# TheCacophonyProject/audio-analysis

Hardware: AMD Instinct MI355X
Metric: audio-seconds classified/sec/GPU on 60 s mono; max|delta logit| vs CPU ref (higher is better)
Workload: dtype bf16x3; 1 GPU; config2: 64 windows/step (39 of clip A + 25 of clip B, 60 s 48 kHz mono), htk log-mel n_fft 4096 hop 640 160 mel + model1 CNN; model=model1, global_batch=64, seq_len=144000, parallelism=dp1, pipeline=2 batches in flight on 2 streams, clip_pairs=4 resident clip pairs in rotation, one per step

## Files before the change

audio-analysis_amd/csrc/aa_cnn.hip:

```cpp
#include "aa_common.h"

#include <cmath>
#include <cstdlib>
#include <cstring>
#include <string>
#include <type_traits>
#include <vector>

namespace aa {

typedef __attribute__((ext_vector_type(8))) __bf16 bf16x8;
typedef __attribute__((ext_vector_type(4))) float f32x4;
typedef __attribute__((ext_vector_type(2))) float f32x2;
typedef __attribute__((ext_vector_type(16))) float f32x16;
typedef __bf16 bf16;
struct fp8 {
    uint8_t v;
};
struct bf16x3 {};

template <typename T>
struct Prec {
    using L = T;
    using G = T;
// ... 801 lines not shown
        for (int dx = 0; dx < pw; ++dx) {
            const int h = oh * ph + dy, x = ow * pw + dx;
            float acc[8];
#pragma unroll
            for (int o = 0; o < 8; ++o) acc[o] = 0.f;
            for (int i = 0; i < kh; ++i)
                for (int j = 0; j < kw; ++j) {
                    const TI* src = img + ((size_t)(h + i) * Win + x + j) * cin;
                    const float* wk = w + (size_t)c0 * K + (i * kw + j) * cin;
                    for (int c = 0; c < cin; ++c) {
                        float v = to_f(src[c]);
                        if (has_mag) v = powf(v, mag_exp);
#pragma unroll
                        for (int o = 0; o < 8; ++o)
                            if (o < nc) acc[o] = fmaf(v, wk[(size_t)o * K + c], acc[o]);
                    }
                }
#pragma unroll
            for (int o = 0; o < 8; ++o)
                if (o < nc) best[o] = fmaxf(best[o], apply_act(acc[o] + bias[c0 + o], act, alpha));
        }
    TO* dst = out + ((size_t)(n * Hout + oh) * Wout + ow) * cout + c0;
    for (int o = 0; o < nc; ++o) dst[o] = to_t<TO>(best[o]);
}

template <typename TI>
__global__ __launch_bounds__(256) void pool_dense(const TI* __restrict__ in, int HW, int C,
                                                  const float* __restrict__ w, const float* __restrict__ b, int U,
                                                  int sigmoid, float* __restrict__ logits, float* __restrict__ probs) {
    extern __shared__ float mx[];
    const int n = blockIdx.x;
    const TI* src = in + (size_t)n * HW * C;
    for (int c = threadIdx.x; c < C; c += blockDim.x) {
        float m = -INFINITY;
        for (int p = 0; p < HW; ++p) m = fmaxf(m, to_f(src[(size_t)p * C + c]));
        mx[c] = m;
    }
    __syncthreads();
    for (int u = threadIdx.x; u < U; u += blockDim.x) {
        float v;
        if (w) {
            v = 0.f;
            for (int c = 0; c < C; ++c) v = fmaf(mx[c], w[(size_t)c * U + u], v);
            v += b[u];
        } else {
            v = mx[u];
        }
        logits[(size_t)n * U + u] = v;
        if (probs) probs[(size_t)n * U + u] = sigmoid ? 1.f / (1.f + expf(-v)) : v;
    }
}

__global__ void track_mean(const float* __restrict__ probs, int n_models, long long model_stride, int L,
                           const int* __restrict__ wb, const int* __restrict__ wc,
                           float* __restrict__ out) {
    const int t = blockIdx.x;
    const int c = threadIdx.x;
    if (c >= L) return;
    constexpr int U = 40;
    float acc = 0.f;
    const int n = wc[t];
    const float* base = probs + (size_t)wb[t] * L + c;
    for (int w0 = 0; w0 < n; w0 += U) {
        float m[U];
#pragma unroll
        for (int u = 0; u < U; ++u) m[u] = 0.f;
        for (int k = 0; k < n_models; ++k) {
            float v[U];
#pragma unroll
            for (int u = 0; u < U; ++u) v[u] = base[k * model_stride + (size_t)min(w0 + u, n - 1) * L];
#pragma unroll
            for (int u = 0; u < U; ++u) m[u] = __fadd_rn(m[u], v[u]);
        }
#pragma unroll
        for (int u = 0; u < U; ++u)
            if (w0 + u < n) acc = __fadd_rn(acc, __fdiv_rn(m[u], (float)n_models));
    }
    out[(size_t)t * L + c] = n > 0 ? __fdiv_rn(acc, (float)n) : NAN;
}

}

#include "aa_conv_x3.h"
#include "aa_conv_wg.h"
#include "aa_gconv.h"
#include "aa_conv_tail.h"

namespace aa {

template <int MODE>
__global__ void stage_decode(const void* __restrict__ src, float* __restrict__ dst, size_t total, int cout) {
    for (size_t i = (size_t)blockIdx.x * blockDim.x + threadIdx.x; i < total; i += (size_t)gridDim.x * blockDim.x) {
        float v;
        if (MODE == 0) {
            v = static_cast<const float*>(src)[i];
        } else if (MODE == 1) {
            v = __uint_as_float((uint32_t) static_cast<const uint16_t*>(src)[i] << 16);
        } else if (MODE == 2) {
            const uint32_t b = static_cast<const uint8_t*>(src)[i];
            const int e = (b >> 3) & 15, m = b & 7;
            const float a = (e == 15 && m == 7) ? __uint_as_float(0x7fc00000u)
                            : e == 0            ? ldexpf((float)m, -9)
                                                : ldexpf((float)(8 + m), e - 10);
            v = (b & 0x80) ? -a : a;
        } else {
            const size_t pix = i / (size_t)cout;
            const int c = (int)(i - pix * (size_t)cout);
            const uint16_t* h = static_cast<const uint16_t*>(src) + pix * (size_t)cout * 2 + (size_t)(c >> 5) * 64 + (c & 31);
            v = __uint_as_float((uint32_t)h[0] << 16) + __uint_as_float((uint32_t)h[32] << 16);
        }
        dst[i] = v;
    }
}

}

#include "aa_cnn_plan.h"

namespace aa {

template <typename Launch>
static int launch_tuned(const Stage& s, const Stage* first, int n, const void* kernel, size_t lds, bool window32,
                        int pool, int th, int tw, int bn, Launch&& launch) {
    if (window32)
        AA_CHECK((double)s.Hin * s.Win * s.cin * 4 < 2147483647.0, AA_ERR_UNSUPPORTED,
                 "conv %s: one window's activations exceed 2 GiB", s.name.c_str());
    FirstConv fc{};
    if (first) {
        const float slope = first->act == ACT_LEAKY ? first->alpha : first->act == ACT_RELU ? 0.f : 1.f;
        fc = FirstConv{(const float*)first->d_w, first->d_b, first->act, slope, first->has_mag,
                       first->mag_exp, first->Hin, first->Win, s.lm_f16};
    }
    AA_CHECK(lds <= 160 * 1024, AA_ERR_UNSUPPORTED, "conv %s: %zu B LDS", s.name.c_str(), lds);
    AA_DYN_LDS(kernel, lds);
    const int tiles_h = (s.Hout * pool + th - 1) / th;
    const int tiles_w = (s.Wout * pool + tw - 1) / tw;
    launch(dim3(tiles_h * tiles_w, s.cout_pad / bn, n), tiles_w, fc);
    AA_LAUNCH_CHECK();
    return AA_OK;
}

template <typename T, int KH, int KW, int CIN, int WM, int WN, int MF, int NF, int POOL, int TH, int TW,
          bool FUSED = false, bool EBF16 = false, int OCC = 0>
static int launch_mfma(const Stage& s, const void* in, void* out, int n, hipStream_t st,
                       const Stage* first = nullptr) {
    auto k = conv_mfma<T, KH, KW, CIN, WM, WN, MF, NF, POOL, TH, TW, FUSED, 0, EBF16, OCC>;
    constexpr int BN = WN * NF * 16;
    const size_t lds = conv_lds_bytes<T, KH, KW, CIN, BN, TH, TW, FUSED, EBF16>();
    using GT = typename Prec<T>::G;
    using LT = typename Prec<T>::L;
    return launch_tuned(s, FUSED ? first : nullptr, n, (const void*)k, lds, false, POOL, TH, TW, BN,
                        [&](dim3 grid, int tiles_w, const FirstConv& fc) {
        hipLaunchKernelGGL(k, grid, dim3(WM * WN * 64), lds, st, (const GT*)in, s.Hin, s.Win, (const LT*)s.d_w, s.d_b,
                           (GT*)out, s.Hout, s.Wout, s.cout, tiles_w, s.act, s.alpha, fc);
    });
}

template <int KH, int KW, int CIN, int WM, int WN, int MF, int NF, int POOL, int TH, int TW, bool RING, bool AJIT,
          int OCC, bool FUSED, bool IN_SPLIT, bool OUT_SPLIT>
static int launch_x3(const Stage& s, const void* in, void* out, int n, hipStream_t st, const Stage* first) {
    auto k = conv_x3<KH, KW, CIN, WM, WN, MF, NF, POOL, TH, TW, FUSED, 0, RING, AJIT, OCC, IN_SPLIT, OUT_SPLIT>;
    constexpr int BN = WN * NF * 16;
    const size_t lds = x3_lds_bytes<KH, KW, CIN, BN, TH, TW, FUSED, RING>();
    return launch_tuned(s, FUSED ? first : nullptr, n, (const void*)k, lds, true, POOL, TH, TW, BN,
                        [&](dim3 grid, int tiles_w, const FirstConv& fc) {
        hipLaunchKernelGGL(k, grid, dim3(WM * WN * 64), lds, st, (const float*)in, s.Hin, s.Win, (const bf16*)s.d_w,
                           s.d_b, (float*)out, s.Hout, s.Wout, s.cout, tiles_w, s.act, s.alpha, fc);
    });
}

template <int KH, int CIN, int WM, int WN, int MF, int NF, int POOL, int TH, int TW, int OCC, int WO, int NPASS,
          int BD, int SLIDE, bool IN_SPLIT, bool OUT_SPLIT>
static int launch_wg(const Stage& s, const void* in, void* out, int n, hipStream_t st) {
    auto k = conv_wg<KH, CIN, WM, WN, MF, NF, POOL, TH, TW, OCC, IN_SPLIT, OUT_SPLIT, 0, WO, NPASS, BD, SLIDE>;
    constexpr int BN = WN * NF * 16;
    const size_t lds = wg_lds_bytes<KH, BN, TH, TW, WO, NPASS, WN>();
    return launch_tuned(s, nullptr, n, (const void*)k, lds, true, POOL, TH, TW, BN,
                        [&](dim3 grid, int tiles_w, const FirstConv&) {
        hipLaunchKernelGGL(k, grid, dim3(WM * WN * 64), lds, st, (const float*)in, s.Hin, s.Win, (const bf16*)s.d_w,
                           s.d_b, (float*)out, s.Hout, s.Wout, s.cout, tiles_w, s.act, s.alpha);
    });
}

template <bool CAN_FUSE, typename F>
static int dispatch_split(const Stage& s, F&& f) {
    using Y = std::true_type;
    using N = std::false_type;
    if constexpr (CAN_FUSE) {
        if (s.fused_first) return s.out_split ? f(Y{}, N{}, Y{}) : f(Y{}, N{}, N{});
    }
    if (s.in_split) return s.out_split ? f(N{}, Y{}, Y{}) : f(N{}, Y{}, N{});
    return s.out_split ? f(N{}, N{}, Y{}) : f(N{}, N{}, N{});
}

template <typename T>
static int launch_stage(const Model& m, const Stage& s, const void* in, void* out, float* logits,
                        float* probs, int n, hipStream_t st, const Stage* first, float* tmp) {
    using GT = typename Prec<T>::G;
    if (s.kind == ST_SMALL) {
        dim3 grid((s.Hc * s.Wc + 255) / 256, n);
        hipLaunchKernelGGL((conv_small<GT, 3, 3, 32>), grid, dim3(256), 0, st, (const float*)in, s.Hin,
                           s.Win, (const float*)s.d_w, s.d_b, s.has_mag, s.mag_exp, (GT*)out, s.Hc, s.Wc,
                           s.act, s.alpha);
        AA_LAUNCH_CHECK();
        return AA_OK;
    }
    if (s.kind == ST_GCONV) {
        if constexpr (!is_split<T>()) {
            set_error("%s: the runtime-shaped MFMA conv is split-bf16 only", s.name.c_str());
            return AA_ERR_UNSUPPORTED;
        } else {
            const ConvGeom g{s.Hin, s.Win, s.cin, s.Hc, s.Wc, s.cout, s.kh, s.kw, 1, 1, 0, 0, s.cin_pad};
            const bool pooled = s.ph > 1 || s.pw > 1;
            float* conv_out = pooled ? tmp : static_cast<float*>(out);
            const int gact_ = s.act == ACT_LEAKY ? GACT_LEAKY : s.act == ACT_RELU ? GACT_RELU : GACT_NONE;
            hipLaunchKernelGGL((gconv_x3t<2, 2, 2, 2>), dim3((s.Hc * s.Wc + 63) / 64, s.cout_pad / 64, n), dim3(256), 0, st,
                               (const float*)in, (const uint16_t*)s.d_w, s.d_b, conv_out, g, s.cout_pad, gact_,
                               s.alpha, nullptr, nullptr);
            AA_LAUNCH_CHECK();
            if (pooled) {
                const size_t items = (size_t)s.Hout * s.Wout * s.cout;
                hipLaunchKernelGGL(gpool2d, dim3((unsigned)((items + 255) / 256), n), dim3(256), 0, st, tmp,
                                   (float*)out, s.Hc, s.Wc, s.cout, s.Hout, s.Wout, s.ph, s.pw, s.ph, s.pw, 0, 0, 0,
                                   GACT_NONE, 0.f);
                AA_LAUNCH_CHECK();
            }
            return AA_OK;
        }
    }
    if (s.kind == ST_GENERIC) {
        if constexpr (is_fp8<T>()) {
            set_error("%s: no fp8 kernel for this shape", s.name.c_str());
            return AA_ERR_UNSUPPORTED;
        } else {
            dim3 grid((s.Hout * s.Wout + 255) / 256, (s.cout + 7) / 8, n);
            if (s.is_first) {
                hipLaunchKernelGGL((conv_generic<float, GT>), grid, dim3(256), 0, st, (const float*)in, s.Hin,
                                   s.Win, s.cin, (const float*)s.d_w, s.d_b, s.kh, s.kw, s.cout, s.ph, s.pw, s.Hout,
                                   s.Wout, s.act, s.alpha, s.has_mag, s.mag_exp, (GT*)out);
            } else {
                hipLaunchKernelGGL((conv_generic<GT, GT>), grid, dim3(256), 0, st, (const GT*)in, s.Hin, s.Win,
                                   s.cin, (const float*)s.d_w, s.d_b, s.kh, s.kw, s.cout, s.ph, s.pw, s.Hout,
                                   s.Wout, s.act, s.alpha, 0, 1.f, (GT*)out);
            }
            AA_LAUNCH_CHECK();
            return AA_OK;
        }
    }
    if (s.kind == ST_POOLDENSE) {
        hipLaunchKernelGGL((pool_dense<GT>), dim3(n), dim3(256), (size_t)s.cin * sizeof(float), st, (const GT*)in,
                           s.Hin * s.Win, s.cin, (const float*)s.d_w, s.d_b, s.cout, s.sigmoid, logits, probs);
        AA_LAUNCH_CHECK();
        return AA_OK;
    }
    if (s.kind == ST_HEAD && s.tail) {
        if constexpr (is_split<T>()) {
            const Stage& c = *first;
            const int tiles_h = (c.Hc + TAIL_TH - 1) / TAIL_TH, tiles_w = (c.Wc + TAIL_TW - 1) / TAIL_TW;
            auto k = conv_tail_x3<1, 3, 128, AA_TAIL_MF, TAIL_TH, TAIL_TW>;
            constexpr size_t lds = tail_lds_bytes<1, 3, 128, TAIL_TH, TAIL_TW>();
            AA_DYN_LDS(k, lds);
            float* part = static_cast<float*>(out);
            hipLaunchKernelGGL(k, dim3(tiles_h * tiles_w, 1, n), dim3(TAIL_NW * 64), lds, st, (const float*)in, c.Hin,
                               c.Win, (const bf16*)c.d_w, c.d_b, c.Hc, c.Wc, tiles_w, c.act, c.alpha,
                               (const bf16*)s.d_tw, part);
            AA_LAUNCH_CHECK();
            hipLaunchKernelGGL(head_final, dim3(n), dim3(64), 0, st, part, tiles_h * tiles_w, 32, s.d_b, s.cout, s.act,
                               s.alpha, s.sigmoid, logits, probs, (const float*)nullptr);
            AA_LAUNCH_CHECK();
            return AA_OK;
        } else {
            set_error("%s: the fused tail is split-bf16 only", s.name.c_str());
            return AA_ERR_UNSUPPORTED;
        }
    }
    if (s.kind == ST_HEAD) {
        const int HW = s.Hin * s.Win, parts = (HW + 63) / 64;
        float* part = static_cast<float*>(out);
        const float* hsc = is_fp8<T>() ? s.d_b + s.cout_pad : nullptr;
        hipLaunchKernelGGL((conv_head<GT, 1, 2>), dim3(n, parts, s.cout_pad / 32), dim3(256), 0, st, (const GT*)in,
                           HW, s.cin, (const GT*)s.d_w, s.d_b, s.cout, s.act, s.alpha, s.sigmoid, logits, probs, part,
                           hsc);
        AA_LAUNCH_CHECK();
        hipLaunchKernelGGL(head_final, dim3(n), dim3(s.cout <= 64 ? 64 : 256), 0, st, part, parts, s.cout_pad, s.d_b,
                           s.cout, s.act, s.alpha, s.sigmoid, logits, probs, hsc);
        AA_LAUNCH_CHECK();
        return AA_OK;
    }
    if (s.fused_first) {
        AA_CHECK(s.kh == 3 && s.kw == 3 && s.cin == 32 && s.pool == 3, AA_ERR_UNSUPPORTED,
                 "no fused first-layer kernel for %s", s.name.c_str());
    }
    if constexpr (is_split<T>()) {
        if (s.wg) {
#define AA_LAUNCHW(KH, CIN, POOL, WM, WN, MF, NF, TH, TW, OCC, WO, NPASS, BD, SLIDE)                             \
            if (s.kh == KH && s.cin == CIN && s.pool == POOL)                                                    \
                return dispatch_split<false>(s, [&](auto, auto is, auto os) {                                    \
                    return launch_wg<KH, CIN, WM, WN, MF, NF, POOL, TH, TW, OCC, WO, NPASS, BD, SLIDE,           \
                                     decltype(is)::value, decltype(os)::value>(s, in, out, n, st);               \
                });
            AA_WG_CFGS(AA_LAUNCHW)
#undef AA_LAUNCHW
            set_error("conv %dx%d cin %d pool %d: no Winograd kernel instantiation", s.kh, s.kw, s.cin, s.pool);
            return AA_ERR_UNSUPPORTED;
        }
#define AA_LAUNCH3(KH, KW, CIN, POOL, WM, WN, MF, NF, TH, TW, RING, AJIT, OCC)                                   \
        if (s.kh == KH && s.kw == KW && s.cin == CIN && s.pool == POOL)                                          \
            return dispatch_split<CIN == 32 && KH == 3 && KW == 3>(s, [&](auto fu, auto is, auto os) {           \
                return launch_x3<KH, KW, CIN, WM, WN, MF, NF, POOL, TH, TW, RING, AJIT, OCC, decltype(fu)::value, \
                                 decltype(is)::value, decltype(os)::value>(s, in, out, n, st, first);            \
            });
        AA_X3_CFGS(AA_LAUNCH3)
#undef AA_LAUNCH3
        set_error("conv %dx%d cin %d pool %d: no split-bf16 kernel instantiation", s.kh, s.kw, s.cin, s.pool);
        return AA_ERR_UNSUPPORTED;
    }
#define AA_LAUNCH(T_, KH, KW, CIN, POOL, WM, WN, MF, NF, TH, TW, EB, OCC)                                        \
    if constexpr (std::is_same<T, T_>::value) {                                                          \
        if (s.kh == KH && s.kw == KW && s.cin == CIN && s.pool == POOL) {                                \
            if (s.fused_first) {                                                                         \
                if constexpr (CIN == 32 && KH == 3 && KW == 3)                                           \
                    return launch_mfma<T, KH, KW, CIN, WM, WN, MF, NF, POOL, TH, TW, true, EB, OCC>(s, in, out, \
                                                                                              n, st, first); \
            } else {                                                                                     \
                return launch_mfma<T, KH, KW, CIN, WM, WN, MF, NF, POOL, TH, TW, false, EB, OCC>(s, in, out, n, st); \
            }                                                                                            \
        }                                                                                                \
    }
    AA_CONV_CFGS(AA_LAUNCH)
#undef AA_LAUNCH
    set_error("conv %dx%d cin %d pool %d: no kernel instantiation", s.kh, s.kw, s.cin, s.pool);
    return AA_ERR_UNSUPPORTED;
}

static void free_model(Model* m) {
    if (!m) return;
    m->timer.release();
    if (m->uploaded)
        for (auto& s : m->st) {
            (void)hipFree(s.d_w);
            (void)hipFree(s.d_b);
            (void)hipFree(s.d_tw);
        }
    delete m;
}

static int upload_model(Model* m) {
    m->uploaded = true;
    auto put = [](void** d, const void* h, size_t bytes) {
        hipError_t e = hipMalloc(d, bytes ? bytes : 4);
        if (e == hipSuccess && bytes) e = hipMemcpy(*d, h, bytes, hipMemcpyHostToDevice);
        return e;
    };
    for (Stage& s : m->st) {
        hipError_t e = s.h_w.empty() ? hipSuccess : put(&s.d_w, s.h_w.data(), s.h_w.size());
        if (e == hipSuccess) e = put((void**)&s.d_b, s.h_b.data(), sizeof(float) * s.h_b.size());
        AA_CHECK(e == hipSuccess, AA_ERR_HIP, "aa_model_create: layer %d: %s", s.layer_end, hipGetErrorString(e));
        if (!s.h_tw.empty()) e = put(&s.d_tw, s.h_tw.data(), s.h_tw.size());
        AA_CHECK(e == hipSuccess, AA_ERR_HIP, "aa_model_create: %s", hipGetErrorString(e));
        std::vector<uint8_t>().swap(s.h_w);
        std::vector<uint8_t>().swap(s.h_tw);
        std::vector<float>().swap(s.h_b);
    }
    return AA_OK;
}

template <typename T>
static int run_stages_t(Model* m, const void* x, int n, int last_stage, float* logits, float* probs, void* workspace,
                        hipStream_t st, bool timed, const void** last_out) {
    const size_t es = prec_bytes(m->prec);
    char* buf[2] = {static_cast<char*>(workspace),
                    static_cast<char*>(workspace) + align_up(m->act_elems[0] * es * n, 256)};
    float* tmp = reinterpret_cast<float*>(buf[1] + align_up(m->act_elems[1] * es * n, 256));
    const void* in = x;
    for (int k = 0; k <= last_stage; ++k) {
        const Stage& s = m->st[k];
        if (s.skipped) continue;
        void* out = buf[(s.tail ? k - 1 : k) % 2];
        const Stage* first = (s.fused_first || s.tail) ? &m->st[k - 1] : nullptr;
        hipEvent_t e0 = nullptr;
        int rc = timed ? m->timer.begin(k, st, &e0) : AA_OK;
        if (rc != AA_OK) return rc;
        rc = launch_stage<T>(*m, s, in, out, logits, probs, n, st, first, tmp);
        if (rc != AA_OK) return rc;
        rc = m->timer.end(k, st, e0);
        if (rc != AA_OK) return rc;
        in = out;
    }
    if (last_out) *last_out = in;
    return AA_OK;
}

static int run_stages(Model* m, const void* x, int n, int last_stage, float* logits, float* probs, void* workspace,
                      hipStream_t st, bool timed, const void** last_out = nullptr) {
    switch (m->prec) {
        case AA_PREC_BF16: return run_stages_t<bf16>(m, x, n, last_stage, logits, probs, workspace, st, timed, last_out);
        case AA_PREC_FP8: return run_stages_t<fp8>(m, x, n, last_stage, logits, probs, workspace, st, timed, last_out);
        case AA_PREC_BF16X3: return run_stages_t<bf16x3>(m, x, n, last_stage, logits, probs, workspace, st, timed, last_out);
        default: return run_stages_t<float>(m, x, n, last_stage, logits, probs, workspace, st, timed, last_out);
    }
}

}

using namespace aa;

extern "C" int aa_model_plan(const aa_layer* layers, int32_t n_layers, const float* blob, int64_t blob_len,
                             int32_t in_h, int32_t in_w, int32_t in_c, int32_t precision, void** model) {
    AA_CHECK(model, AA_ERR_INVALID, "aa_model_create: null argument");
    Model* m = nullptr;
    const int rc = plan_model(layers, n_layers, blob, blob_len, in_h, in_w, in_c, precision, &m);
    if (rc == AA_OK) *model = m;
    return rc;
}

extern "C" int aa_model_create(const aa_layer* layers, int32_t n_layers, const float* blob, int64_t blob_len,
                               int32_t in_h, int32_t in_w, int32_t in_c, int32_t precision, void** model) {
    void* m = nullptr;
    int rc = aa_model_plan(layers, n_layers, blob, blob_len, in_h, in_w, in_c, precision, model ? &m : nullptr);
    if (rc != AA_OK) return rc;
    rc = upload_model(static_cast<Model*>(m));
    if (rc != AA_OK) {
        free_model(static_cast<Model*>(m));
        return rc;
    }
    *model = m;
    return AA_OK;
}

extern "C" int aa_model_stage_image(const void* model, int32_t stage, int32_t which, void* buf, size_t cap,
                                    size_t* len) {
// ... 153 lines not shown
```

audio-analysis_amd/csrc/aa_cnn_plan.h:

```cpp
#pragma once

#include <algorithm>
#include <cmath>
#include <string>
#include <vector>

#include "aa_cnn_pack.h"
#include "aa_cnn_tiles.h"

namespace aa {

enum StageKind { ST_SMALL = 0, ST_MFMA = 1, ST_HEAD = 2, ST_GENERIC = 3, ST_POOLDENSE = 4, ST_GCONV = 5 };

struct Stage {
    int kind = ST_MFMA;
    int kh = 1, kw = 1, cin = 0, cout = 0, cout_pad = 0;
    int pool = 1;
    int ph = 1, pw = 1;
    int act = ACT_NONE;
    float alpha = 0.f;
    int has_mag = 0;
    float mag_exp = 1.f;
    int sigmoid = 0;
    int Hin = 0, Win = 0, Hc = 0, Wc = 0, Hout = 0, Wout = 0;
    std::vector<uint8_t> h_w, h_tw;
    std::vector<float> h_b;
    int layer_end = 0;
    void* d_w = nullptr;
    float* d_b = nullptr;
    double flops = 0, bytes = 0;
    std::string name;
    int skipped = 0;
    int is_first = 0;
    int fused_first = 0;
    int lm_f16 = 0;
    int in_split = 0;
    int out_split = 0;
    int wg = 0;
    int wg_npass = 1;
    int cin_pad = 0;
    int tail = 0;
    void* d_tw = nullptr;
};

struct Model {
    int prec = AA_PREC_BF16;
    int in_h = 0, in_w = 0, in_c = 0;
    int L = 0;
    bool uploaded = false;
    std::vector<Stage> st;
    size_t act_elems[2] = {0, 0};
    size_t tmp_elems = 0;
    StageTimer timer;
};

static size_t prec_bytes(int prec) { return prec == AA_PREC_FP8 ? 1 : prec == AA_PREC_BF16 ? 2 : 4; }

struct LayerCursor {
    const aa_layer* layers;
    int n_layers;
    const float* blob;
    int64_t blob_len;
    int prec;
    int i = 0;
    int H = 0, W = 0, C = 0;
    int has_mag = 0;
    float mag_exp = 1.f;

    const float* get(int64_t off, int64_t n) const {
        if (off < 0 || off + n > blob_len) return nullptr;
        return blob + off;
    }
    bool at(int op) const { return i < n_layers && layers[i].op == op; }
    int fail(int code, const char* msg) const {
        set_error("aa_model_create: layer %d: %s", i, msg);
        return code;
    }
};

struct Fold {
    const float* kern = nullptr;
    std::vector<double> scale, shift;
};

static std::string pool_suffix(const Stage& s) {
    char pl[24] = "";
    if (s.ph > 1 || s.pw > 1) snprintf(pl, sizeof pl, s.ph == s.pw ? "_pool%d" : "_pool%dx%d", s.ph, s.pw);
    return pl;
}

static int plan_pooldense(LayerCursor& p, Stage& s) {
    const int C = p.C;
    s.kind = ST_POOLDENSE;
    s.Hin = p.H;
    s.Win = p.W;
    s.cin = C;
    s.cout = C;
    ++p.i;
    std::vector<float> wd;
    if (p.at(AA_OP_DENSE)) {
        const aa_layer& d = p.layers[p.i];
        s.cout = d.filters;
        const float* k = p.get(d.off[0], (int64_t)C * d.filters);
        if (!k || d.filters <= 0) return p.fail(AA_ERR_INVALID, "dense kernel outside the blob");
        wd.assign(k, k + (size_t)C * d.filters);
        s.h_b.assign(d.filters, 0.f);
        if (d.off[1] >= 0) {
            const float* bb = p.get(d.off[1], d.filters);
            if (!bb) return p.fail(AA_ERR_INVALID, "dense bias outside the blob");
            s.h_b.assign(bb, bb + d.filters);
        }
        ++p.i;
    }
    if (p.at(AA_OP_SIGMOID)) {
        s.sigmoid = 1;
        ++p.i;
    }
    if (p.i != p.n_layers) return p.fail(AA_ERR_UNSUPPORTED, "layers after the global pooling / dense");
    s.cout_pad = s.cout;
    s.h_w = pack_rowmajor_f32(wd);
    s.flops = 2.0 * C * (wd.empty() ? 0 : s.cout);
    s.bytes = (double)prec_bytes(p.prec) * p.H * p.W * C + 4.0 * s.cout;
    char nm[96];
    snprintf(nm, sizeof nm, "globalmax%s_%d_%d", wd.empty() ? "" : "_dense", C, s.cout);
    s.name = nm;
    return AA_OK;
}

static int parse_conv(LayerCursor& p, bool first, Stage& s, Fold& f) {
    const aa_layer& ly = p.layers[p.i];
    s.kh = ly.kh;
    s.kw = ly.kw;
    s.cin = p.C;
    s.cout = ly.filters;
    s.Hin = p.H;
    s.Win = p.W;
// ... 268 lines not shown
```

audio-analysis_amd/csrc/aa_cnn_tiles.h:

```cpp
#pragma once

namespace aa {

#define AA_CONV_CFGS(X)                                     \
    X(bf16, 3, 3, 32, 3, 4, 1, 6, 2, 18, 21, true, 0)          \
    X(bf16, 3, 3, 32, 1, 2, 2, 4, 2, 8, 16, true, 0)           \
    X(bf16, 3, 3, 64, 1, 2, 2, 4, 2, 8, 16, true, 0)           \
    X(bf16, 9, 3, 64, 3, 4, 2, 6, 4, 39, 9, true, 0)           \
    X(bf16, 1, 3, 128, 1, 2, 4, 5, 2, 7, 20, false, 0)         \
    X(fp8, 3, 3, 32, 3, 4, 1, 6, 2, 12, 30, true, 0)           \
    X(fp8, 3, 3, 32, 1, 2, 2, 4, 2, 8, 16, true, 0)            \
    X(fp8, 3, 3, 64, 1, 4, 1, 3, 4, 12, 16, true, 0)           \
    X(fp8, 9, 3, 64, 3, 4, 2, 6, 4, 21, 18, true, 0)           \
    X(fp8, 1, 3, 128, 1, 2, 4, 5, 2, 7, 20, true, 0)           \
    X(float, 3, 3, 32, 3, 2, 2, 9, 1, 6, 48, false, 0)         \
    X(float, 3, 3, 32, 1, 1, 4, 9, 1, 6, 24, false, 0)         \
    X(float, 3, 3, 64, 1, 1, 4, 9, 1, 6, 24, false, 0)         \
    X(float, 9, 3, 64, 3, 1, 4, 7, 1, 3, 33, false, 0)         \
    X(float, 1, 3, 128, 1, 2, 2, 5, 1, 6, 24, false, 0)

#ifdef AA_X3_ALT
#define AA_X3_CFGS(X) AA_X3_ALT(X)
#else
#define AA_X3_CFGS(X)                                 \
    X(3, 3, 32, 3, 4, 1, 4, 2, 12, 21, 0, 1, 0)       \
    X(3, 3, 32, 1, 4, 2, 3, 2, 10, 18, 1, 0, 4)       \
    X(3, 3, 64, 1, 2, 2, 3, 2, 12, 8, 1, 1, 0)        \
    X(9, 3, 64, 3, 2, 2, 4, 2, 21, 6, 0, 1, 4)        \
    X(1, 3, 128, 1, 2, 2, 3, 2, 7, 12, 1, 1, 0)
#endif

#ifdef AA_WG_ALT
#define AA_WG_CFGS(X) AA_WG_ALT(X)
#else
#define AA_WG_CFGS(X) X(9, 64, 3, 1, 4, 3, 1, 39, 6, 0, 6, 1, 4, 9)
#endif

#ifndef AA_TAIL_TW
#define AA_TAIL_TW 5
#define AA_TAIL_MF 5
#endif
constexpr int TAIL_TH = 13, TAIL_TW = AA_TAIL_TW;

static int wg_bn(int kh, int kw, int cin, int pool) {
#define AA_WBN(KH, CIN, POOL, WM, WN, MF, NF, TH, TW, OCC, WO, NPASS, BD, SLIDE) \
    if (kw == 3 && kh == KH && cin == CIN && pool == POOL) return WN * NF * 16;
    AA_WG_CFGS(AA_WBN)
#undef AA_WBN
    return 0;
}
static void wg_form(int kh, int cin, int pool, int* wo, int* npass) {
#define AA_WFORM(KH, CIN, POOL, WM, WN, MF, NF, TH, TW, OCC, WO, NPASS, BD, SLIDE) \
    if (kh == KH && cin == CIN && pool == POOL) { *wo = WO; *npass = NPASS; return; }
    AA_WG_CFGS(AA_WFORM)
#undef AA_WFORM
    *wo = 0;
    *npass = 1;
}

template <typename T>
constexpr int prec_of() {
    return is_split<T>() ? AA_PREC_BF16X3 : sizeof(T) == 1 ? AA_PREC_FP8 : sizeof(T) == 2 ? AA_PREC_BF16 : AA_PREC_F32;
}

static int mfma_bn(int prec, int kh, int kw, int cin, int pool) {
    if (prec == AA_PREC_BF16X3 && wg_bn(kh, kw, cin, pool)) return wg_bn(kh, kw, cin, pool);
#define AA_BN(T_, KH, KW, CIN, POOL, WM, WN, MF, NF, TH, TW, EB, OCC)                                       \
    if (prec_of<T_>() == prec && kh == KH && kw == KW && cin == CIN && pool == POOL) \
        return WN * NF * 16;
    AA_CONV_CFGS(AA_BN)
#undef AA_BN
#define AA_BN3(KH, KW, CIN, POOL, WM, WN, MF, NF, TH, TW, RING, AJIT, OCC)                                               \
    if (prec == AA_PREC_BF16X3 && kh == KH && kw == KW && cin == CIN && pool == POOL) return WN * NF * 16;
    AA_X3_CFGS(AA_BN3)
#undef AA_BN3
    return 0;
}

}
```

audio-analysis_amd/csrc/aa_conv_x3.h:

```cpp
#pragma once

namespace aa {

constexpr int X3_CG = 32;

#ifndef AA_X3_XSPLIT
#define AA_X3_XSPLIT 1
#endif
#ifndef AA_X3_REMAP
#define AA_X3_REMAP 1
#endif
#ifndef AA_F1_KPACK
#define AA_F1_KPACK 1
#endif
#ifndef AA_X3_SCALAR_SPLIT
#define AA_X3_SCALAR_SPLIT 1
#endif

#ifndef AA_PIN_X3
#define AA_PIN_X3 3
#endif
#ifndef AA_X3_PRIO
#define AA_X3_PRIO 1
#endif
// ... 516 lines not shown
                        b1.z = __builtin_amdgcn_perm(xv[5], xv[4], psel);
                        b1.w = __builtin_amdgcn_perm(xv[7], xv[6], psel);
                        b2.x = kg ? xv[8] : b1.x;
                        b2.y = kg ? (xv[8] & 0xffffu) : b1.y;
                        b2.z = kg ? 0u : b1.z;
                        b2.w = kg ? 0u : b1.w;
                        xh[u] = __builtin_bit_cast(bf16x8, b1);
                        xl[u] = __builtin_bit_cast(bf16x8, b2);
                    } else if constexpr (AA_X3_XSPLIT) {
                        const uint32_t* xp = Xs + r * XW + c;
                        uint32_t xv[8];
                        xv[0] = xp[off0];
#pragma unroll
                        for (int j = 1; j < 8; ++j) xv[j] = xp[(j / 3) * XW + j % 3];
                        uint4 hh, ll;
                        hh.x = __builtin_amdgcn_perm(xv[1], xv[0], 0x05040100u);
                        hh.y = __builtin_amdgcn_perm(xv[3], xv[2], 0x05040100u);
                        hh.z = __builtin_amdgcn_perm(xv[5], xv[4], 0x05040100u);
                        hh.w = __builtin_amdgcn_perm(xv[7], xv[6], 0x05040100u);
                        ll.x = __builtin_amdgcn_perm(xv[1], xv[0], 0x07060302u);
                        ll.y = __builtin_amdgcn_perm(xv[3], xv[2], 0x07060302u);
                        ll.z = __builtin_amdgcn_perm(xv[5], xv[4], 0x07060302u);
                        ll.w = __builtin_amdgcn_perm(xv[7], xv[6], 0x07060302u);
                        xh[u] = __builtin_bit_cast(bf16x8, hh);
                        xl[u] = __builtin_bit_cast(bf16x8, ll);
                    } else {
                        const float* xp = X + r * XW + c;
                        float xv[8];
                        xv[0] = xp[off0];
#pragma unroll
                        for (int j = 1; j < 8; ++j) xv[j] = xp[(j / 3) * XW + j % 3];
#pragma unroll
                        for (int j = 0; j < 8; ++j) {
                            xh[u][j] = bf_hi(xv[j]);
                            xl[u][j] = bf_lo(xv[j]);
                        }
                    }
                }
                f32x16 d[NU];
                if constexpr (DIAG & 8192) {
#pragma unroll
                    for (int u = 0; u < NU; ++u) {
                        d[u] = cb;
                        d[u][0] += __builtin_bit_cast(float, __builtin_bit_cast(uint4, xh[u]).x ^ __builtin_bit_cast(uint4, xl[u]).y);
                    }
                } else if constexpr (AA_F1_KPACK) {
#pragma unroll
                    for (int u = 0; u < NU; ++u) d[u] = __builtin_amdgcn_mfma_f32_32x32x16_bf16(wa, xh[u], cb, 0, 0, 0);
#pragma unroll
                    for (int u = 0; u < NU; ++u) d[u] = __builtin_amdgcn_mfma_f32_32x32x16_bf16(wal, xl[u], d[u], 0, 0, 0);
                } else {
#pragma unroll
                for (int u = 0; u < NU; ++u) d[u] = __builtin_amdgcn_mfma_f32_32x32x16_bf16(wa, xh[u], cb, 0, 0, 0);
#pragma unroll
                for (int u = 0; u < NU; ++u) d[u] = __builtin_amdgcn_mfma_f32_32x32x16_bf16(wa, xl[u], d[u], 0, 0, 0);
#pragma unroll
                for (int u = 0; u < NU; ++u) d[u] = __builtin_amdgcn_mfma_f32_32x32x16_bf16(wal, xh[u], d[u], 0, 0, 0);
                }
#pragma unroll
                for (int u = 0; u < NU; ++u) {
                    if ((g0 + NW * u) * 32 + l32 < NPX) {
                        const int R = pix[u] / PW, C = pix[u] - R * PW;
#pragma unroll
                        for (int h = 0; h < 2; ++h) {
                            uint32_t hw[4], lw[4];
#pragma unroll
                            for (int e = 0; e < 8; e += 2) {
                                if constexpr (DIAG & 16384) {
                                    hw[e >> 1] = __builtin_bit_cast(uint32_t, d[u][8 * h + e]);
                                    lw[e >> 1] = __builtin_bit_cast(uint32_t, d[u][8 * h + e + 1]);
                                } else {
                                    leaky_split2(d[u][8 * h + e], d[u][8 * h + e + 1], ae, hw[e >> 1], lw[e >> 1]);
                                }
                            }
                            const int a = x3_addr(R, C, 2 * kg + h, PW, TW);
                            if ((DIAG & 32768) && hw[0] != 0x12345u) continue;
                            *reinterpret_cast<uint4*>(patch + a) = make_uint4(hw[0], hw[1], hw[2], hw[3]);
                            *reinterpret_cast<uint4*>(patch + (a ^ 64)) = make_uint4(lw[0], lw[1], lw[2], lw[3]);
                        }
                    }
                }
            }
        }
        if constexpr (DIAG & 4096) ts[6] = __builtin_amdgcn_s_memtime();

        if (g == 0) {
            if constexpr (RING && !(DIAG & 32)) {
                if (hi_share) wait_vm_lgkm<GHI>(min(NB - 2, NSTEP - 1));
                else wait_vm_lgkm<GLO>(min(NB - 2, NSTEP - 1));
            }
        }
        __syncthreads();
        if (g == 0) {
            if constexpr (RING) read_b(F0, 0);
        }
        else if constexpr ((NTAP - 1) % 2 == 0) {
#pragma unroll
            for (int j = 0; j < NF; ++j) {
                F0.bh[j] = F1.bh[j];
                F0.bl[j] = F1.bl[j];
            }
        }
        if (!(DIAG & 2) && !AJIT) read_a(F0, 0);
        const bool wave_idle = !RING && oh0 + (wm * MF * 16) / TW >= Hout * POOL;
        if constexpr (DIAG & 4096) ts[1] = __builtin_amdgcn_s_memtime();
        if constexpr (AA_X3_PRIO > 0) __builtin_amdgcn_s_setprio(AA_X3_PRIO);
#pragma unroll
        for (int t = 0; t < ((DIAG & 2) || wave_idle ? 0 : NTAP); t += 2) {
            step(F0, F1, g, t);
            if (t + 1 < NTAP) step(F1, F0, g, t + 1);
        }
        if constexpr (AA_X3_PRIO > 0) __builtin_amdgcn_s_setprio(0);
        if constexpr (DIAG & 4096) ts[2] = __builtin_amdgcn_s_memtime();
    }
#undef X3_GLDS
    __syncthreads();

    float* E = reinterpret_cast<float*>(smem);
#pragma unroll
    for (int j = 0; j < NF; ++j) {
        const int u = wn * NF * 4 + j * 4 + q;
#pragma unroll
        for (int i = 0; i < MF; ++i) {
            const int p = (wm * MF + i) * 16 + (lane & 15);
            if (p < TH * TW)
                *reinterpret_cast<float4*>(E + x3_eoff<BN, 0>(p, u)) =
                    make_float4(acc[i][j][0], acc[i][j][1], acc[i][j][2], acc[i][j][3]);
        }
    }
    __syncthreads();
    x3_store<TH, TW, POOL, BN, NTHR, OUT_SPLIT, (DIAG & 4) != 0, 0>(E, bias, out, n, cb, oh0, ow0, Hout, Wout,
                                                                  cout_store, act, alpha);
    if constexpr (DIAG & 4096) {
        ts[3] = __builtin_amdgcn_s_memtime();
        if (lane == 0) {
            const int L = blockIdx.x + gridDim.x * (blockIdx.y + gridDim.y * blockIdx.z);
            unsigned long long* d = reinterpret_cast<unsigned long long*>(out + (64u << 20)) + ((size_t)L * NW + wave0) * 10;
            for (int k = 0; k < 8; ++k) d[k] = ts[k];
            d[8] = __builtin_amdgcn_s_getreg((31 << 11) | 4);
            d[9] = __builtin_amdgcn_s_getreg((15 << 11) | 20);
        }
    }
}

}
```

Before: 278,700 audio-s/s.

## Add persistent pipelined split-bf16 conv kernel for 3x3 cin64 pool1 layers

```diff
diff --git a/audio-analysis_amd/csrc/aa_cnn.hip b/audio-analysis_amd/csrc/aa_cnn.hip
--- a/audio-analysis_amd/csrc/aa_cnn.hip
+++ b/audio-analysis_amd/csrc/aa_cnn.hip
@@ -907,6 +907,7 @@
 }
 
 #include "aa_conv_x3.h"
+#include "aa_conv_x3p.h"
 #include "aa_conv_wg.h"
 #include "aa_gconv.h"
 #include "aa_conv_tail.h"
@@ -994,6 +995,26 @@
     });
 }
 
+template <int KH, int KW, int CIN, int WM, int WN, int MF, int NF, int TH, int TW, int NB, int BPC, bool APRE,
+          bool OUT_SPLIT>
+static int launch_x3p(const Model& m, const Stage& s, const void* in, void* out, int n, hipStream_t st) {
+    auto k = conv_x3p<KH, KW, CIN, WM, WN, MF, NF, TH, TW, NB, BPC, OUT_SPLIT, APRE>;
+    constexpr int BN = WN * NF * 16;
+    const size_t lds = x3p_lds_bytes<KH, KW, BN, TH, TW, NB>();
+    AA_CHECK((double)s.Hout * s.Wout * s.cout * 4 < 2147483647.0, AA_ERR_UNSUPPORTED,
+             "conv %s: one window's output exceeds 2 GiB", s.name.c_str());
+    return launch_tuned(s, nullptr, n, (const void*)k, lds, true, 1, TH, TW, BN,
+                        [&](dim3 grid, int tiles_w, const FirstConv&) {
+        const long long items = (long long)grid.x * n;
+        long long blocks = (long long)BPC * m.cu_count;
+        if (m.x3p_cap > 0 && blocks > m.x3p_cap) blocks = m.x3p_cap;
+        if (blocks > items) blocks = items;
+        hipLaunchKernelGGL(k, dim3((unsigned)blocks), dim3(WM * WN * 64), lds, st, (const float*)in, s.Hin, s.Win,
+                           (const bf16*)s.d_w, s.d_b, (float*)out, s.Hout, s.Wout, s.cout, tiles_w, (int)grid.x,
+                           (int)items, s.act, s.alpha);
+    });
+}
+
 template <int KH, int CIN, int WM, int WN, int MF, int NF, int POOL, int TH, int TW, int OCC, int WO, int NPASS,
           int BD, int SLIDE, bool IN_SPLIT, bool OUT_SPLIT>
 static int launch_wg(const Stage& s, const void* in, void* out, int n, hipStream_t st) {
@@ -1129,6 +1150,15 @@
             set_error("conv %dx%d cin %d pool %d: no Winograd kernel instantiation", s.kh, s.kw, s.cin, s.pool);
             return AA_ERR_UNSUPPORTED;
         }
+#if AA_X3P
+#define AA_LAUNCH3P(KH, KW, CIN, WM, WN, MF, NF, TH, TW, NB, BPC, APRE)                                          \
+        if (s.kh == KH && s.kw == KW && s.cin == CIN && s.pool == 1 && s.in_split && !s.fused_first &&           \
+            s.cout == WN * NF * 16 && s.cout_pad == WN * NF * 16 && n > 0 && (long long)n * s.Hout * s.Wout < (1 << 30)) \
+            return s.out_split ? launch_x3p<KH, KW, CIN, WM, WN, MF, NF, TH, TW, NB, BPC, APRE != 0, true>(m, s, in, out, n, st) \
+                               : launch_x3p<KH, KW, CIN, WM, WN, MF, NF, TH, TW, NB, BPC, APRE != 0, false>(m, s, in, out, n, st);
+        AA_X3P_CFGS(AA_LAUNCH3P)
+#undef AA_LAUNCH3P
+#endif
 #define AA_LAUNCH3(KH, KW, CIN, POOL, WM, WN, MF, NF, TH, TW, RING, AJIT, OCC)                                   \
         if (s.kh == KH && s.kw == KW && s.cin == CIN && s.pool == POOL)                                          \
             return dispatch_split<CIN == 32 && KH == 3 && KW == 3>(s, [&](auto fu, auto is, auto os) {           \
@@ -1172,6 +1202,15 @@
 
 static int upload_model(Model* m) {
     m->uploaded = true;
+    {
+        int dev = 0, cus = 0;
+        hipError_t e = hipGetDevice(&dev);
+        if (e == hipSuccess) e = hipDeviceGetAttribute(&cus, hipDeviceAttributeMultiprocessorCount, dev);
+        AA_CHECK(e == hipSuccess && cus > 0, AA_ERR_HIP, "aa_model_create: compute unit count: %s", hipGetErrorString(e));
+        m->cu_count = cus;
+        const char* cap = getenv("AA_X3P_MAX_BLOCKS");
+        m->x3p_cap = cap ? atoi(cap) : 0;
+    }
     auto put = [](void** d, const void* h, size_t bytes) {
         hipError_t e = hipMalloc(d, bytes ? bytes : 4);
         if (e == hipSuccess && bytes) e = hipMemcpy(*d, h, bytes, hipMemcpyHostToDevice);
diff --git a/audio-analysis_amd/csrc/aa_cnn_plan.h b/audio-analysis_amd/csrc/aa_cnn_plan.h
--- a/audio-analysis_amd/csrc/aa_cnn_plan.h
+++ b/audio-analysis_amd/csrc/aa_cnn_plan.h
@@ -52,6 +52,7 @@
     size_t act_elems[2] = {0, 0};
     size_t tmp_elems = 0;
     StageTimer timer;
+    int cu_count = 0, x3p_cap = 0;
 };
 
 static size_t prec_bytes(int prec) { return prec == AA_PREC_FP8 ? 1 : prec == AA_PREC_BF16 ? 2 : 4; }
diff --git a/audio-analysis_amd/csrc/aa_cnn_tiles.h b/audio-analysis_amd/csrc/aa_cnn_tiles.h
--- a/audio-analysis_amd/csrc/aa_cnn_tiles.h
+++ b/audio-analysis_amd/csrc/aa_cnn_tiles.h
@@ -28,6 +28,13 @@
     X(3, 3, 64, 1, 2, 2, 3, 2, 12, 8, 1, 1, 0)        \
     X(9, 3, 64, 3, 2, 2, 4, 2, 21, 6, 0, 1, 4)        \
     X(1, 3, 128, 1, 2, 2, 3, 2, 7, 12, 1, 1, 0)
+#endif
+
+#ifdef AA_X3P_ALT
+#define AA_X3P_CFGS(X) AA_X3P_ALT(X)
+#else
+#define AA_X3P_CFGS(X) \
+    X(3, 3, 64, 2, 2, 3, 2, 12, 8, 3, 2, 1)
 #endif
 
 #ifdef AA_WG_ALT
diff --git a/audio-analysis_amd/csrc/aa_conv_x3.h b/audio-analysis_amd/csrc/aa_conv_x3.h
--- a/audio-analysis_amd/csrc/aa_conv_x3.h
+++ b/audio-analysis_amd/csrc/aa_conv_x3.h
@@ -622,7 +622,8 @@
                 }
             }
         }
-        if constexpr (DIAG & 4096) ts[6] = __builtin_amdgcn_s_memtime();
+        const bool ts_g0 = !FUSED && NG > 1 && g == 0;
+        if constexpr (DIAG & 4096) ts[ts_g0 ? 4 : 6] = __builtin_amdgcn_s_memtime();
 
         if (g == 0) {
             if constexpr (RING && !(DIAG & 32)) {
@@ -643,7 +644,7 @@
         }
         if (!(DIAG & 2) && !AJIT) read_a(F0, 0);
         const bool wave_idle = !RING && oh0 + (wm * MF * 16) / TW >= Hout * POOL;
-        if constexpr (DIAG & 4096) ts[1] = __builtin_amdgcn_s_memtime();
+        if constexpr (DIAG & 4096) ts[ts_g0 ? 5 : 1] = __builtin_amdgcn_s_memtime();
         if constexpr (AA_X3_PRIO > 0) __builtin_amdgcn_s_setprio(AA_X3_PRIO);
 #pragma unroll
         for (int t = 0; t < ((DIAG & 2) || wave_idle ? 0 : NTAP); t += 2) {
@@ -651,7 +652,7 @@
             if (t + 1 < NTAP) step(F1, F0, g, t + 1);
         }
         if constexpr (AA_X3_PRIO > 0) __builtin_amdgcn_s_setprio(0);
-        if constexpr (DIAG & 4096) ts[2] = __builtin_amdgcn_s_memtime();
+        if constexpr (DIAG & 4096) ts[ts_g0 ? 7 : 2] = __builtin_amdgcn_s_memtime();
     }
 #undef X3_GLDS
     __syncthreads();
diff --git a/audio-analysis_amd/csrc/aa_conv_x3p.h b/audio-analysis_amd/csrc/aa_conv_x3p.h
--- /dev/null
+++ b/audio-analysis_amd/csrc/aa_conv_x3p.h
@@ -0,0 +1,284 @@
+#pragma once
+
+namespace aa {
+
+#ifndef AA_X3P
+#define AA_X3P 1
+#endif
+
+template <int KH, int KW, int TH, int TW>
+__host__ __device__ constexpr int x3p_patch_bytes() {
+    return (TH + KH - 1) * (TW + KW - 1) * 128;
+}
+template <int KH, int KW, int BN, int TH, int TW, int NB>
+constexpr size_t x3p_lds_bytes() {
+    return 2 * (size_t)x3p_patch_bytes<KH, KW, TH, TW>() + (size_t)NB * BN * 128;
+}
+
+__device__ __forceinline__ void x3p_wait(int n) {
+#define AA_W(K) case K: asm volatile("s_waitcnt vmcnt(%0) lgkmcnt(0)" ::"n"(K) : "memory"); break;
+#define AA_W8(K) AA_W(K) AA_W(K + 1) AA_W(K + 2) AA_W(K + 3) AA_W(K + 4) AA_W(K + 5) AA_W(K + 6) AA_W(K + 7)
+    switch (n) { AA_W8(0) AA_W8(8) AA_W8(16) AA_W8(24) AA_W8(32) AA_W8(40) AA_W8(48) default: AA_W(56) }
+#undef AA_W8
+#undef AA_W
+}
+
+template <int NTAP, int NB, int NW, int NCH, int GSH, int NSTORE>
+struct X3pSched {
+    static constexpr int R = (NCH + NW - 1) / NW;
+    static constexpr int TP = NTAP - NB + 2;
+    static constexpr int RPS = (R + TP - 1) / TP;
+    static constexpr bool PARTIAL = NCH % NW != 0;
+    static_assert(NB >= 3 && NB - 2 <= NTAP, "ring depth");
+    static_assert(TP >= 1 && RPS * TP >= R, "patch rounds fit before the next unit's first ring share");
+    static constexpr int r0(int t) { return t * RPS < R ? t * RPS : R; }
+    static constexpr int r1(int t) { return (t + 1) * RPS < R ? (t + 1) * RPS : R; }
+    static constexpr int count(int t, bool first, bool full) {
+        int n = (NB - 3) * GSH;
+        for (int k = 1; k <= NB - 2; ++k) {
+            const int tt = ((t - k) % NTAP + NTAP) % NTAP;
+            n += r1(tt) - r0(tt);
+            if (PARTIAL && !full && r0(tt) <= R - 1 && R - 1 < r1(tt)) --n;
+        }
+        if (first && t < NB - 2) n += NSTORE;
+        return n;
+    }
+};
+
+template <int KH, int KW, int CIN, int WM, int WN, int MF, int NF, int TH, int TW, int NB, int BPC, bool OUT_SPLIT,
+          bool APRE = false>
+__global__ __launch_bounds__(WM * WN * 64) __attribute__((amdgpu_waves_per_eu(1, (BPC * WM * WN + 3) / 4 > 8 ? 8 : (BPC * WM * WN + 3) / 4)))
+void conv_x3p(const float* __restrict__ in, int Hin, int Win, const bf16* __restrict__ wt,
+              const float* __restrict__ bias, float* __restrict__ out, int Hout, int Wout, int cout_store,
+              int tiles_w, int tiles, int items, int act, float alpha) {
+#if defined(__HIP_DEVICE_COMPILE__)
+    static_assert(TH * TW <= WM * MF * 16, "tile covered by the waves' fragments");
+    static_assert(CIN % X3_CG == 0, "C_in multiple of 32");
+    static_assert((KW - 1) % 2 == 0, "odd kernel width (the swizzle needs even row jumps)");
+    constexpr int BN = WN * NF * 16;
+    constexpr int PH = TH + KH - 1, PW = TW + KW - 1;
+    constexpr int NTAP = KH * KW, NG = CIN / X3_CG, NSTEP = NTAP * NG;
+    static_assert(NTAP % 2 == 1, "an odd tap count: the fragment sets swap once per unit");
+    constexpr int NW = WM * WN;
+    constexpr int SLICE = BN * 64;
+    constexpr int SLICE_LDS = BN * 128;
+    constexpr int GPS = SLICE_LDS / 1024;
+    static_assert(GPS % NW == 0, "every wave loads the same share of a slice");
+    constexpr int GSH = GPS / NW;
+    constexpr int PATCHB = x3p_patch_bytes<KH, KW, TH, TW>();
+    constexpr int UNITS = PH * PW * 8;
+    constexpr int NCH = (UNITS + 63) / 64;
+    constexpr int NSTORE = MF * NF * (OUT_SPLIT ? 2 : 1);
+    using SCH = X3pSched<NTAP, NB, NW, NCH, GSH, NSTORE>;
+    constexpr int R = SCH::R;
+    extern __shared__ __attribute__((aligned(16))) char smem[];
+    char* Bs = smem + 2 * PATCHB;
+
+    const int G = gridDim.x, b = blockIdx.x;
+    int first = b, stride = G, end = items;
+    if (AA_X3_REMAP != 0 && (G & 7) == 0) {
+        const int x = b & 7;
+        first = (int)((long long)items * x / 8) + (b >> 3);
+        end = (int)((long long)items * (x + 1) / 8);
+        stride = G >> 3;
+    }
+    if (first >= end) return;
+    const int wave0 = __builtin_amdgcn_readfirstlane(threadIdx.x >> 6);
+    const int lane = threadIdx.x & 63;
+
+    const __amdgpu_buffer_rsrc_t wrs = x3_wrsrc(wt);
+#define X3P_GLDS(slot, sl)                                                                                  \
+    _Pragma("unroll") for (int u_ = 0; u_ < GSH; ++u_) {                                                  \
+        const int g_ = u_ * NW + wave0;                                                                     \
+        __builtin_amdgcn_raw_ptr_buffer_load_lds(                                                          \
+            wrs, (__attribute__((address_space(3))) void*)(Bs + (slot) * SLICE_LDS + g_ * 1024), 16, lane * 16, \
+            __builtin_amdgcn_readfirstlane((int)(((sl) * SLICE + g_ * 512) * 2)), 0, 0);                   \
+    }
+#pragma unroll
+    for (int s = 0; s < NB - 1; ++s) { X3P_GLDS(s, s % NSTEP) }
+
+    int pR[R], pC[R], pU[R];
+#pragma unroll
+    for (int r = 0; r < R; ++r) {
+        const int idx = min((r * NW + wave0) * 64 + lane, UNITS - 1);
+        const int pix = idx >> 3, slot = idx & 7;
+        pR[r] = pix / PW;
+        pC[r] = pix - pR[r] * PW;
+        pU[r] = ((slot - pR[r] * TW - pC[r]) & 7) * 16;
+    }
+    const bool p_last = !SCH::PARTIAL || (R - 1) * NW + wave0 < NCH;
+    struct Pos {
+        int n, oh0, ow0;
+    };
+    auto locate = [&](int it) {
+        const int n = it / tiles, tile = it - n * tiles;
+        const int th = tile / tiles_w, tw = tile - th * tiles_w;
+        return Pos{n, th * TH, tw * TW};
+    };
+    auto stage = [&](const Pos& ps, int g, int buf, int ra, int rb) {
+        const __amdgpu_buffer_rsrc_t ars = x3_wrsrc(reinterpret_cast<const char*>(in) + (size_t)ps.n * Hin * Win * CIN * 4);
+#pragma unroll
+        for (int r = ra; r < rb; ++r) {
+            const int ch = r * NW + wave0;
+            if (r + 1 < R || p_last) {
+                if (ch * 64 + lane < UNITS) {
+                    const int gh = min(ps.oh0 + pR[r], Hin - 1), gw = min(ps.ow0 + pC[r], Win - 1);
+                    __builtin_amdgcn_raw_ptr_buffer_load_lds(
+                        ars, (__attribute__((address_space(3))) void*)(smem + buf * PATCHB + ch * 1024), 16,
+                        (gh * Win + gw) * (CIN * 4) + pU[r], g * 128, 0, 0);
+                }
+            }
+        }
+    };
+    Pos cur = locate(first);
+    stage(cur, 0, 0, 0, R);
+
+    const int wave = wave0, wm = wave % WM, wn = wave / WM;
+    const int q = lane >> 4;
+    int abase[MF], aph[MF], opix[MF];
+#pragma unroll
+    for (int i = 0; i < MF; ++i) {
+        int p = (wm * MF + i) * 16 + (lane & 15);
+        opix[i] = p < TH * TW ? ((p / TW) << 16) | (p - (p / TW) * TW) : -1;
+        if (p >= TH * TW) p = max(p - 16 * ((p - TH * TW) / 16 + 1), 0);
+        const int r = p / TW, c = p - (p / TW) * TW;
+        abase[i] = (r * PW + c) * 128;
+        aph[i] = p + q;
+    }
+    int bofs[NF];
+    float4 bq[NF];
+#pragma unroll
+    for (int j = 0; j < NF; ++j) {
+        const int row = wn * NF * 16 + j * 16 + (lane & 15);
+        bofs[j] = row * 128 + (((q + row) & 7) << 4);
+        bq[j] = *reinterpret_cast<const float4*>(bias + wn * NF * 16 + j * 16 + q * 4);
+    }
+
+    f32x4 acc[MF][NF];
+#pragma unroll
+    for (int i = 0; i < MF; ++i)
+#pragma unroll
+        for (int j = 0; j < NF; ++j) acc[i][j] = f32x4{0.f, 0.f, 0.f, 0.f};
+
+    struct BSet {
+        bf16x8 bh[NF], bl[NF];
+    };
+    BSet F0, F1;
+    auto read_b = [&](BSet& f, int slot) {
+        const char* bsl = Bs + slot * SLICE_LDS;
+#pragma unroll
+        for (int j = 0; j < NF; ++j) {
+            f.bh[j] = *reinterpret_cast<const bf16x8*>(bsl + bofs[j]);
+            f.bl[j] = *reinterpret_cast<const bf16x8*>(bsl + (bofs[j] ^ 64));
+        }
+    };
+
+    asm volatile("s_waitcnt vmcnt(0) lgkmcnt(0)" ::: "memory");
+#pragma unroll
+    for (int j = 0; j < NF; ++j) asm volatile("" : "+v"(bq[j].x), "+v"(bq[j].y), "+v"(bq[j].z), "+v"(bq[j].w));
+    __builtin_amdgcn_s_barrier();
+    __builtin_amdgcn_sched_barrier(0);
+    read_b(F0, 0);
+
+    int slot = 0;
+    int pb = 0;
+    bf16x8 h2[2], l2[2];
+    auto step = [&](BSet& fc, BSet& fn, const int* ab, int g, int t, const Pos& np, int ng) {
+        if (p_last) x3p_wait(SCH::count(t, g == 0, true));
+        else x3p_wait(SCH::count(t, g == 0, false));
+        __builtin_amdgcn_s_barrier();
+        __builtin_amdgcn_sched_barrier(0);
+        {
+            const int ls = slot == 0 ? NB - 1 : slot - 1;
+            X3P_GLDS(ls, (g * NTAP + t + NB - 1) % NSTEP)
+        }
+        if (SCH::r0(t) < SCH::r1(t)) stage(np, ng, pb ^ 1, SCH::r0(t), SCH::r1(t));
+        slot = slot + 1 == NB ? 0 : slot + 1;
+        read_b(fn, slot);
+        auto rd = [&](int tt, int i) {
+            const int kh = tt / KW, kw = tt - (tt / KW) * KW;
+            const int toff = (kh * PW + kw) * 128, tv = kh * TW + kw;
+            const int a = ab[i] + toff + (((aph[i] + tv) & 7) << 4), k = (tt * MF + i) & 1;
+            h2[k] = *reinterpret_cast<const bf16x8*>(smem + a);
+            l2[k] = *reinterpret_cast<const bf16x8*>(smem + (a ^ 64));
+        };
+        if (!APRE || t == 0) rd(t, 0);
+#pragma unroll
+        for (int i = 0; i < MF; ++i) {
+            if (i + 1 < MF) rd(t, i + 1);
+            else if (APRE && t + 1 < NTAP) rd(t + 1, 0);
+            const int k = (t * MF + i) & 1;
+#pragma unroll
+            for (int j = 0; j < NF; ++j) {
+                acc[i][j] = __builtin_amdgcn_mfma_f32_16x16x32_bf16(fc.bh[j], h2[k], acc[i][j], 0, 0, 0);
+                acc[i][j] = __builtin_amdgcn_mfma_f32_16x16x32_bf16(fc.bl[j], h2[k], acc[i][j], 0, 0, 0);
+                acc[i][j] = __builtin_amdgcn_mfma_f32_16x16x32_bf16(fc.bh[j], l2[k], acc[i][j], 0, 0, 0);
+            }
+        }
+    };
+
+    const size_t owin = (size_t)Hout * Wout * cout_store * 4;
+    for (int it = first; it < end; it += stride) {
+        const Pos nxt = locate(it + stride < end ? it + stride : it);
+        if constexpr (AA_X3_PRIO > 0) __builtin_amdgcn_s_setprio(AA_X3_PRIO);
+#pragma unroll
+        for (int g = 0; g < NG; ++g) {
+            int ab[MF];
+#pragma unroll
+            for (int i = 0; i < MF; ++i) ab[i] = abase[i] + pb * PATCHB;
+            const Pos& up = g + 1 < NG ? cur : nxt;
+            const int ug = g + 1 < NG ? g + 1 : 0;
+#pragma unroll
+            for (int t = 0; t < NTAP; t += 2) {
+                step(F0, F1, ab, g, t, up, ug);
+                if (t + 1 < NTAP) step(F1, F0, ab, g, t + 1, up, ug);
+            }
+#pragma unroll
+            for (int j = 0; j < NF; ++j) {
+                F0.bh[j] = F1.bh[j];
+                F0.bl[j] = F1.bl[j];
+            }
+            pb ^= 1;
+        }
+        if constexpr (AA_X3_PRIO > 0) __builtin_amdgcn_s_setprio(0);
+
+        const int n = cur.n, oh0 = cur.oh0, ow0 = cur.ow0;
+        const __amdgpu_buffer_rsrc_t ors = __builtin_amdgcn_make_buffer_rsrc(
+            reinterpret_cast<char*>(out) + (size_t)n * owin, 0, (int)owin, 0x00020000);
+#pragma unroll
+        for (int i = 0; i < MF; ++i) {
+            const int gh = oh0 + (opix[i] >> 16), gw = ow0 + (opix[i] & 0xffff);
+            const bool ok = opix[i] >= 0 && gh < Hout && gw < Wout;
+            const int pofs = (gh * Wout + gw) * cout_store * 4;
+#pragma unroll
+            for (int j = 0; j < NF; ++j) {
+                const int ch0 = wn * NF * 16 + j * 16 + q * 4;
+                float4 v;
+                v.x = apply_act(acc[i][j][0] + bq[j].x, act, alpha);
+                v.y = apply_act(acc[i][j][1] + bq[j].y, act, alpha);
+                v.z = apply_act(acc[i][j][2] + bq[j].z, act, alpha);
+                v.w = apply_act(acc[i][j][3] + bq[j].w, act, alpha);
+                acc[i][j] = f32x4{0.f, 0.f, 0.f, 0.f};
+                typedef __attribute__((ext_vector_type(4))) unsigned int u32x4;
+                typedef __attribute__((ext_vector_type(2))) unsigned int u32x2;
+                if constexpr (OUT_SPLIT) {
+                    const int o = ok ? pofs + (ch0 >> 5) * 128 + (ch0 & 31) * 2 : (int)owin;
+                    uint32_t h0, l0, h1, l1;
+                    split2(v.x, v.y, h0, l0);
+                    split2(v.z, v.w, h1, l1);
+                    __builtin_amdgcn_raw_buffer_store_b64(u32x2{h0, h1}, ors, o, 0, 0);
+                    __builtin_amdgcn_raw_buffer_store_b64(u32x2{l0, l1}, ors, ok ? o + 64 : (int)owin, 0, 0);
+                } else {
+                    const int o = ok ? pofs + ch0 * 4 : (int)owin;
+                    __builtin_amdgcn_raw_buffer_store_b128(__builtin_bit_cast(u32x4, v), ors, o, 0, 0);
+                }
+            }
+        }
+        cur = nxt;
+    }
+#undef X3P_GLDS
+    asm volatile("s_waitcnt vmcnt(0)" ::: "memory");
+#endif
+}
+
+}
```

New measurement: 277,000 audio-s/s. No clear change (-0.6%).
